# VatsalSy/gerris-fft-particles

Hardware: AMD Instinct MI355X
Metric: Mcell-steps/s (projection+advection), 3D 256^3 uniform (higher is better)
Workload: dtype f64; 1 GPU; 3-D periodic Taylor-Green, 256^3 per GPU, default projection/advection parameters (SURVEY 8d config C); relax_mode=exact, parallelism=1 box, rccl_world_size=0

## Files before the change

gerris-fft-particles_amd/csrc/gfship_internal.hpp:

```cpp
#pragma once

#include <hip/hip_runtime.h>
#include <cstdio>
#include <cstdarg>
#include <cstring>
#include <vector>
#include <deque>
#include <string>
#include <type_traits>
#include "gfship.h"
#include "switches.hpp"
#include "cell_update.hpp"

namespace gfship {

struct Layout {
  int n = 0;
  int px = 0;
  int xo = 1;
  int rows = 0;
  int dim = 3;
  long sy = 0;
  long sz = 0;
  size_t total = 0;
// ... 195 lines not shown
			const RelaxOp * op = nullptr);
int launch_relax_mpi_first (gfship_domain * dom, unsigned dimension, int level, double omega,
			    double * u, const double * rhs, const double * dia, const RelaxOp * op,
			    int (* after_shell) (void *), void * ctx);
void mpi_order_free (gfship_domain * dom);
int launch_relax_loop_small (gfship_domain * dom, unsigned dimension, int level, double omega,
			     Field * dp, Field * ubc, const double * rhs, const double * dia,
			     unsigned nrelax, bool * done, const RelaxOp * op = nullptr);
int coarse_cycle_top (gfship_domain * dom, int minlevel);
int lattice_cycle_top (gfship_domain * dom, int minlevel, Field * dia);
int lattice_check_error (gfship_domain * dom);
int launch_lattice_cycle (gfship_domain * dom, unsigned dimension, double omega, int lmin, int ltop,
			  const unsigned * nrelax, Field * dp, Field * ubc, Field * res);
int launch_coarse_cycle (gfship_domain * dom, unsigned dimension, double omega, int lmin, int ltop,
			 const unsigned * nrelax, Field * dp, Field * ubc, Field * res, Field * dia);
int launch_relax_redblack (gfship_domain * dom, unsigned dimension, int level, double omega,
			   double * u, const double * rhs, const double * dia);
int launch_residual (gfship_domain * dom, int level, const double * u, const double * rhs,
		     const double * dia, double * res);
int launch_residual_weighted (gfship_domain * dom, int level, const double * u, const double * rhs,
			      const double * dia, double * res);
int launch_poisson_weights (gfship_domain * dom, double * const alpha[3]);
int launch_diffusion_weights (gfship_domain * dom, double * const D[3], double cdt);
int alloc_weights (gfship_domain * dom);
RelaxOp weighted_op (gfship_domain * dom, int level);
int launch_restrict (gfship_domain * dom, unsigned dimension, int level_coarse, double * v_coarse,
		     const double * v_fine);
int launch_prolongate (gfship_domain * dom, int level_coarse, const double * v_coarse,
		       double * v_fine);
int launch_correct (gfship_domain * dom, int level, double * u, const double * dp);
int launch_fill (gfship_domain * dom, int level, double * a, double value);
int launch_residual_norm (gfship_domain * dom, int level, const double * u, const double * rhs,
			  const double * dia, double * res, double scale, double weight,
			  double * out , bool dia_zero = false);
int launch_norm_async (gfship_domain * dom, int level, const double * a, double scale, double weight);
int launch_norm (gfship_domain * dom, int level, const double * a, double scale, double weight,
		 double out[5] );

int launch_face_interp_un (gfship_domain * dom, double * const u[3], double * const un[3]);
int launch_divergence (gfship_domain * dom, double * const un[3], double * div, double dt);
int launch_correct_un (gfship_domain * dom, const double * p, double * const un[3], double dt);
int launch_centered_gradient (gfship_domain * dom, const double * p, double * const g[3]);
int launch_correct_centered (gfship_domain * dom, double * const u[3], double * const g[3], double dt);
int launch_correct_centered_coarse (gfship_domain * dom, double * const u[3], double * const g[3],
				    double dt, double * const uc[3]);
int launch_coarse_init_from (gfship_domain * dom, Field * const * v, int nf, int top);
int launch_coarse_init_levels (gfship_domain * dom, Field * const * v, int nf, int top, int bottom);
int launch_advected_face_values (gfship_domain * dom, const double * v, double * const u[3],
				 double * const un[3], double dt, int use_centered, int gradient,
				 double * const fv[6], int cmask, double visc = 0., double gsrc = 0.,
				 const double * msrc = nullptr );
int launch_variable_mac_source (gfship_domain * dom, const double * v, double * const D[3],
				const double * alpha, double * out);
int launch_mac_source_fields (gfship_domain * dom, int c, const double * F, bool add_out, double * out);
int launch_centered_source_fields (gfship_domain * dom, double * v, const double * F, double gsrc, double dt);
int launch_face_bc (gfship_domain * dom, Field * v, double * const fv[6], int cmask);
int launch_predict_un (gfship_domain * dom, int cc, const double * uc, double * const fv[6],
		       double * unc);
int launch_flux_update (gfship_domain * dom, bool velocity, double * v, double * const un[3],
			double * const fv[6], const double * gm, const double * gc, double dt,
			double gsrc = 0.);
int launch_cfl (gfship_domain * dom, double * const u[3], double * const un[3],
		const double visc[3], double * cfl2,
		double * const msrc[3] = nullptr );
int launch_coarse_init (gfship_domain * dom, Field * const * v, int nf);
int launch_velocity_divergence (gfship_domain * dom, double * const u[3], double * out);
bool godunov_fused_supported (const gfship_domain * dom);
bool godunov_fused_mpi_supported (const gfship_domain * dom);
// ... 63 lines not shown
```

gerris-fft-particles_amd/csrc/poisson.hip:

```cpp
#include "gfship_internal.hpp"
#include <cmath>
#include <cfloat>
#include <cstdlib>

using namespace gfship;

#define GFSHIP_CHECK_DIMENSION(dom, d) \
  GFSHIP_CHECK ((d) == (unsigned) (dom)->dim, GFSHIP_EUNSUPPORTED, \
		"dimension %u on a %d-D domain: only the dimension of the domain is implemented", (d), (dom)->dim)

namespace gfship {

static bool weighted_pipelinable (gfship_domain * dom, unsigned dimension, int level)
{
  return dom->relax_mode == GFSHIP_RELAX_EXACT && dimension == 3 && dom->dim == 3 &&
    skew_supported (dom, level) && !dom->force_hyperplane;
}

static bool weighted_pipelined (gfship_domain * dom, unsigned dimension, int level)
{
  return dom->sw.weighted_pipelined && weighted_pipelinable (dom, dimension, level);
}

static int relax_level (gfship_domain * dom, unsigned dimension, int level, double omega,
// ... 84 lines not shown
    if (done)
      return GFSHIP_OK;
  }
  auto sweep = [&] () -> int {
    if (dom->relax_mode == GFSHIP_RELAX_EXACT && dom->has_external) {
      bool done = false;
      int rr = launch_relax_loop_small (dom, dimension, level, omega, dp, u, rhs->lev[level],
					dia->lev[level], 1, &done);
      if (rr || done) return rr;
    }
    return relax_level (dom, dimension, level, omega, dp, rhs, dia);
  };
  if ((r = launch_bc (dom, u, dp, level, 1))) return r;
  for (unsigned n = 0; n < nrelax - 1; n++) {
    if ((r = sweep ())) return r;
    if ((r = launch_bc (dom, u, dp, level, 1))) return r;
  }
  return sweep ();
}

static int norm_residual_finish (gfship_domain * dom, double dt, double s[5], gfship_norm * out);

static int norm_residual (gfship_domain * dom, double dt, Field * res, gfship_norm * out)
{
  const Layout & L = dom->lay[dom->depth];
  double size = 1./L.n;
  double s[5];
  int r = launch_norm (dom, dom->depth, res->lev[dom->depth], 1.*size*size, 1., s);
  if (r) return r;
  return norm_residual_finish (dom, dt, s, out);
}

static int residual_and_norm (gfship_domain * dom, double dt, Field * U, Field * R, Field * D,
			      Field * S, gfship_norm * out)
{
  const int L = dom->depth;
  S->zero[L] = false;
  if (dom->weighted) {
    int rr = launch_residual_weighted (dom, L, U->lev[L], R->lev[L], D->lev[L], S->lev[L]);
    if (rr) return rr;
    return norm_residual (dom, dt, S, out);
  }
  const double size = 1./dom->lay[L].n;
  double s[5];
  int r = launch_residual_norm (dom, L, U->lev[L], R->lev[L], D->lev[L], S->lev[L], 1.*size*size, 1., s,
				D->zero[L]);
  if (r) return r;
  return norm_residual_finish (dom, dt, s, out);
}

static int norm_residual_finish (gfship_domain * dom, double dt, double s[5], gfship_norm * out)
{
  const Layout & L = dom->lay[dom->depth];
  int r;
  double w = (double) ncells (L);
  if (dom->has_external) {
    double sums[5] = { s[0], s[1], s[2], w, s[4] }, mx[1] = { s[3] };
    if ((r = call_reduce_norm (dom, sums, 5, mx))) return r;
    s[0] = sums[0]; s[1] = sums[1]; s[2] = sums[2]; w = sums[3]; s[3] = mx[0]; s[4] = sums[4];
  }
  gfship_norm n;
  n.bias = s[0]; n.first = s[1]; n.second = s[2]; n.infty = s[3]; n.w = w;
  if (n.w > 0.) {
    n.bias /= n.w;
    n.first /= n.w;
    n.second = sqrt (n.second/n.w);
  }
  else
    n.infty = 0.;
  dt *= dt;
  n.bias = s[4]*dt;
  n.first *= dt;
  n.second *= dt;
  n.infty *= dt;
  *out = n;
  return GFSHIP_OK;
}

}
// ... 100 lines not shown
{
  Field * V = get_field (dom, v);
  if (!V || !out) return GFSHIP_EINVAL;
  const Layout & L = dom->lay[dom->depth];
  double size = 1./L.n;
  double vol = dom->dim == 3 ? size*size*size : size*size;
  double s[5];
  int r = launch_norm (dom, dom->depth, V->lev[dom->depth], 1., vol, s);
  if (r) return r;
  gfship_norm n;
  double wv = vol*(double) ncells (L);
  if (dom->has_external) {
    double sums[4] = { s[0], s[1], s[2], wv }, mx[1] = { s[3] };
    if ((r = call_reduce_norm (dom, sums, 4, mx))) return r;
    s[0] = sums[0]; s[1] = sums[1]; s[2] = sums[2]; wv = sums[3]; s[3] = mx[0];
  }
  n.bias = s[0]; n.first = s[1]; n.second = s[2]; n.infty = s[3];
  n.w = wv;
  if (n.w > 0.) {
    n.bias /= n.w;
    n.first /= n.w;
    n.second = sqrt (n.second/n.w);
  }
  else
    n.infty = 0.;
  *out = n;
  return GFSHIP_OK;
}

}

static int poisson_cycle (gfship_domain * dom, gfship_multilevel_params * p,
			  gfship_field u, gfship_field rhs, gfship_field dia, gfship_field res,
			  double dt, gfship_norm * norm)
{
  GFSHIP_CHECK (dom && p, GFSHIP_EINVAL, "null argument");
  GFSHIP_CHECK (p->dimension == 2 || p->dimension == 3, GFSHIP_EINVAL, "dimension must be 2 or 3");
  GFSHIP_CHECK_DIMENSION (dom, p->dimension);
  GFSHIP_CHECK (p->nrelax > 0 && p->erelax > 0, GFSHIP_EINVAL, "nrelax and erelax must be non zero");
  GFSHIP_CHECK (dom->unit_weights, GFSHIP_EINVAL, "call gfship_poisson_coefficients first");
  if (dom->dp_cache < 0)
    dom->dp_cache = gfship_field_alloc (dom, -1);
  gfship_field dpf = dom->dp_cache;
  if (dpf < 0) return dpf;
  Field * U = get_field (dom, u), * R = get_field (dom, rhs), * D = get_field (dom, dia),
    * S = get_field (dom, res), * DP = get_field (dom, dpf);
  int r = GFSHIP_OK;
  bool corrected = false;
  if (!U || !R || !D || !S) return GFSHIP_EINVAL;
  const int L = dom->depth;
  unsigned minlevel = p->minlevel;
  if (minlevel > (unsigned) L) minlevel = L;
  p->depth = L;

#define TRY(x) do { if ((r = (x)) != GFSHIP_OK) goto done; } while (0)
  for (int l = 0; l <= L; l++)
    S->zero[l] = U->zero[l] = false;
  {
    unsigned nrl[GFSHIP_MAXLEVEL + 1];
    {
      unsigned nr = p->nrelax;
      for (int l = L; l >= 0; l--) {
	nrl[l] = nr;
	if (l > (int) minlevel) nr *= p->erelax;
      }
    }
    for (int l = 0; l <= L; l++)
// ... 15 lines not shown
    unsigned first = minlevel;
    if (ltop >= 0) {
      TRY (launch_lattice_cycle (dom, p->dimension, p->omega, (int) minlevel, ltop, nrl, DP, U, S));
      first = ltop + 1;
    }
    else if (ctop >= 0) {
      TRY (launch_coarse_cycle (dom, p->dimension, p->omega, (int) minlevel, ctop, nrl, DP, U, S, D));
      first = ctop + 1;
    }
    else {
      TRY (launch_fill (dom, minlevel, DP->lev[minlevel], 0.));
      TRY (relax_loop (dom, DP, U, p->dimension, minlevel, p->omega, S, D, nrl[minlevel]));
      first = minlevel + 1;
      dom->kc[GFSHIP_KC_COARSE_END_BY_LEVEL]++;
    }
    for (unsigned l = first; l <= p->depth; l++) {
      const bool fp = prolongation_fused (dom, p->dimension, (int) l, nrl[l]) ||
	line_prolongation_fused (dom, p->dimension, (int) l, nrl[l]);
      if (fp) dom->kc[GFSHIP_KC_PROLONGATION_FUSED]++;
      else if (prolongation_fusable (dom, p->dimension, (int) l, nrl[l]) ||
	       line_prolongation_fusable (dom, p->dimension, (int) l, nrl[l]))
	dom->kc[GFSHIP_KC_PROLONGATION_DECLINED]++;
      if (!fp)
	TRY (launch_prolongate (dom, l - 1, DP->lev[l - 1], DP->lev[l]));
      TRY (relax_loop (dom, DP, U, p->dimension, l, p->omega, S, D, nrl[l],
		       (int) l == L ? U->lev[L] : nullptr, &corrected, fp ? DP->lev[l - 1] : nullptr));
    }
  }
  if (!corrected)
    TRY (launch_correct (dom, L, U->lev[L], DP->lev[L]));
  if (!(corrected && all_sides_periodic (dom)))
    TRY (launch_bc (dom, U, U, L, 0));
  if (norm)
    TRY (residual_and_norm (dom, dt, U, R, D, S, norm));
  else if (dom->weighted)
    TRY (launch_residual_weighted (dom, L, U->lev[L], R->lev[L], D->lev[L], S->lev[L]));
  else
    TRY (launch_residual (dom, L, U->lev[L], R->lev[L], D->lev[L], S->lev[L]));
#undef TRY
 done:
  for (int l = 0; l <= L; l++)
    dom->skew[l].rs_ready = false;
  return r;
}

extern "C" {

int gfship_poisson_cycle (gfship_domain * dom, gfship_multilevel_params * p,
			  gfship_field u, gfship_field rhs, gfship_field dia, gfship_field res)
{
  GFSHIP_CHECK (dom != nullptr, GFSHIP_EINVAL, "null domain");
  int r = before_write (dom);
  if (r) return r;
  return poisson_cycle (dom, p, u, rhs, dia, res, 1., nullptr);
}

int gfship_poisson_solve (gfship_domain * dom, gfship_multilevel_params * par,
			  gfship_field lhs, gfship_field rhs, gfship_field res,
			  gfship_field dia, double dt)
{
  GFSHIP_CHECK (dom && par, GFSHIP_EINVAL, "null argument");
  Field * U = get_field (dom, lhs), * R = get_field (dom, rhs), * D = get_field (dom, dia),
    * S = get_field (dom, res);
  if (!U || !R || !D || !S) return GFSHIP_EINVAL;
  GFSHIP_CHECK (par->dimension == 2 || par->dimension == 3, GFSHIP_EINVAL, "dimension must be 2 or 3");
  GFSHIP_CHECK_DIMENSION (dom, par->dimension);
  GFSHIP_CHECK (dom->unit_weights, GFSHIP_EINVAL, "call gfship_poisson_coefficients first");
  { int r = before_write (dom); if (r) return r; }
  int r;
  const int L = dom->depth;
  if ((r = coarse_flush (dom, U, L, true))) return r;
  unsigned minlevel = par->minlevel;
  par->depth = L;
  par->niter = 0;

  bool deferred = par->nitermin >= 1 && par->nitermax >= 1;
  if (deferred) {
    const Layout & Ly = dom->lay[L];
    double size = 1./Ly.n;
    S->zero[L] = false;
    if (dom->weighted) {
      if ((r = launch_residual_weighted (dom, L, U->lev[L], R->lev[L], D->lev[L], S->lev[L]))) return r;
      if ((r = launch_norm_async (dom, L, S->lev[L], 1.*size*size, 1.))) return r;
    }
    else if ((r = launch_residual_norm (dom, L, U->lev[L], R->lev[L], D->lev[L], S->lev[L], 1.*size*size,
					1., nullptr, D->zero[L])))
      return r;
  }
  else {
    if ((r = residual_and_norm (dom, dt, U, R, D, S, &par->residual))) return r;
    par->residual_before = par->residual;
  }

  double res_max_before = par->residual.infty;

  while (par->niter < par->nitermin ||
	 (par->residual.infty > par->tolerance && par->niter < par->nitermax)) {
    if ((r = poisson_cycle (dom, par, lhs, rhs, dia, res, dt, &par->residual))) {
      if (deferred) {
	deferred = false;
	double s0[5];
	if (hipStreamSynchronize (dom->stream) == hipSuccess) {
	  memcpy (s0, dom->h_pinned + 8, sizeof (s0));
	  if (norm_residual_finish (dom, dt, s0, &par->residual_before) == GFSHIP_OK)
	    par->residual = par->residual_before;
	}
	else
	  memset (&par->residual_before, 0, sizeof (par->residual_before)),
	    memset (&par->residual, 0, sizeof (par->residual));
      }
      break;
    }
    if (deferred) {
      deferred = false;
      double s0[5];
      memcpy (s0, dom->h_pinned + 8, sizeof (s0));
      if ((r = norm_residual_finish (dom, dt, s0, &par->residual_before))) break;
      res_max_before = par->residual_before.infty;
    }
    if (par->residual.infty == res_max_before)
      break;
    if (par->residual.infty > res_max_before/1.1 && par->minlevel < par->depth)
      par->minlevel++;
    res_max_before = par->residual.infty;
    par->niter++;
  }

  par->minlevel = minlevel;
  if (r == GFSHIP_OK)
    r = skew_check_error (dom);
  if (r == GFSHIP_OK)
    r = lattice_check_error (dom);
  return r;
}

int gfship_time_relax (gfship_domain * dom, unsigned d, int level, gfship_field u,
		       gfship_field rhs, gfship_field dia, int reps, double * ms_per_sweep)
{
  Field * U = get_field (dom, u), * R = get_field (dom, rhs), * D = get_field (dom, dia);
  if (!U || !R || !D || !ms_per_sweep || reps <= 0) return GFSHIP_EINVAL;
  GFSHIP_CHECK (level >= 0 && level <= dom->depth, GFSHIP_EINVAL, "level %d out of range", level);
  int r;
  if (dom->relax_mode == GFSHIP_RELAX_EXACT && d == 3 && skew_supported (dom, level) &&
      !dom->force_hyperplane) {
    U->zero[level] = false;
    r = skew_time_sweeps (dom, level, U, R->lev[level], D->lev[level], D->zero[level], reps,
			  ms_per_sweep);
    if (r == GFSHIP_OK && dom->sw.skew_stats)
      skew_dump_stats (dom, level);
    return r;
  }
  if ((r = relax_level (dom, d, level, 1., U, R, D))) return r;
  GFSHIP_HIP (hipEventRecord (dom->ev0, dom->stream));
  for (int q = 0; q < reps; q++)
    if ((r = relax_level (dom, d, level, 1., U, R, D))) return r;
  GFSHIP_HIP (hipEventRecord (dom->ev1, dom->stream));
  GFSHIP_HIP (hipEventSynchronize (dom->ev1));
  float ms = 0.f;
  GFSHIP_HIP (hipEventElapsedTime (&ms, dom->ev0, dom->ev1));
  *ms_per_sweep = (double) ms/reps;
  if (dom->sw.skew_stats)
    skew_dump_stats (dom, level);
  return GFSHIP_OK;
}

int gfship_time_relax_loop (gfship_domain * dom, int level, gfship_field u, gfship_field rhs,
			    gfship_field dia, unsigned nrelax, int reps, double * ms_per_loop,
			    int * fused)
// ... 25 lines not shown
```

gerris-fft-particles_amd/csrc/poisson_kernels.hip:

```cpp
#include "gfship_internal.hpp"
#include "cell_loop.hpp"
#include "relax_skew.hpp"
#include <algorithm>
#include <cstdlib>

namespace gfship {

template <int DIM, int OP>
__device__ __forceinline__ double relax_value (const double * __restrict__ u, long c, long sy, long sz,
					       double rhs, double dia, unsigned dimension,
					       double omega, double w, double h2, const W6 * wf = nullptr)
{
  return cell_update<DIM, OP> (kind_weights<OP> (w, ArrayW { wf, c }), ArrayU { u, c, sy, sz }, rhs, dia, u + c,
			       dimension, omega, h2);
}

__device__ __forceinline__ double relax_value_six (const double * __restrict__ u, long c, long sy, long sz,
						    double rhs)
{
  return cell_update_six (ArrayU { u, c, sy, sz }, rhs);
}

template <int DIM, int OP>
__global__ void __launch_bounds__(256)
// ... 273 lines not shown
  const Layout & L = dom->lay[level];
  BcDesc bc;
  for (int d = 0; d < 6; d++) {
    bc.side[d] = dom->side[d];
    bc.type[d] = ubc->bc[d];
    bc.val[d] = nullptr;
  }
  bc.component = ubc->component;
  bc.homogeneous = 1;
  int nface = dom->dim == 3 ? L.n*L.n : L.n;
  int block = nface <= 64 ? 64 : nface <= 256 ? 256 : 1024;
  with_kind ([&] (auto K, auto D3) {
    hipLaunchKernelGGL ((relax_loop_lds_kernel<decltype (D3)::value ? 3 : 2, decltype (K)::value>), dim3 (1),
			dim3 (block), bytes, dom->stream, L, bc, dimension, omega, w, h2, nrelax, dp->lev[level],
			rhs, dia, op_weights (op));
  }, kind, dom->dim == 3);
  GFSHIP_HIP (hipGetLastError ());
  *done = true;
  return GFSHIP_OK;
}

struct CoarseCycleArgs {
  Layout lay[GFSHIP_MAXLEVEL + 1];
  int lmin, ltop;
  unsigned nrelax[GFSHIP_MAXLEVEL + 1];
  double * dp[GFSHIP_MAXLEVEL + 1];
  double * res[GFSHIP_MAXLEVEL + 2];
  const double * dia[GFSHIP_MAXLEVEL + 1];
  BcDesc bc;
  unsigned dimension;
  double omega;
};

template <int DIM>
__global__ void __launch_bounds__(1024)
coarse_cycle_kernel (CoarseCycleArgs A)
{
  extern __shared__ double lds[];
  const int tid = threadIdx.x, nt = blockDim.x;
#ifdef GFSHIP_LAB_CLOCK
  unsigned long long stamp[40]; int nstamp = 0;
#define LAB_STAMP() do { if (nstamp < 40) stamp[nstamp++] = wall_clock64 (); } while (0)
#else
#define LAB_STAMP() do { } while (0)
#endif
  LAB_STAMP ();
  auto lds_off = [&] (int l, int which) -> unsigned {
    unsigned o = 0;
    for (int q = A.lmin; q < l; q++) {
      unsigned r = A.lay[q].n + 2;
      o += 2*(DIM == 3 ? r*r*r : r*r);
    }
    if (which) {
      unsigned r = A.lay[l].n + 2;
      o += DIM == 3 ? r*r*r : r*r;
    }
    return o;
  };
  {
    const unsigned o = lds_off (A.ltop + 1, 0);
    for (size_t q = tid; q < o; q += nt)
      lds[q] = 0.;
  }
  __syncthreads ();
  LAB_STAMP ();
  for (int l = A.ltop; l >= A.lmin; l--) {
    const Layout & Lc = A.lay[l], & Lf = A.lay[l + 1];
    const int n = Lc.n, r = n + 2, rf = 2*n + 2;
    const int ncell = DIM == 3 ? n*n*n : n*n;
    const bool top = l == A.ltop;
    const double * gf = A.res[l + 1];
    const double * sf = lds + (top ? 0 : lds_off (l + 1, 1));
    double * sc = lds + lds_off (l, 1);
    for (int q = tid; q < ncell; q += nt) {
      int i = q % n + 1, j = (q / n) % n + 1, k = DIM == 3 ? q / (n*n) + 1 : 0;
      double val = 0.;
#pragma unroll
      for (int id = 0; id < (1 << DIM); id++) {
	int ci = 2*i - 1 + (id & 1);
	int cj = 2*j - 1 + ((id & 2) ? 0 : 1);
	int ck = DIM == 3 ? 2*k - 1 + ((id & 4) ? 0 : 1) : 0;
	if (top)
	  val += gf[Lf.idx (ci, cj, ck)];
	else
	  val += sf[ci + rf*(cj + (DIM == 3 ? rf*ck : 0))];
      }
      double v = A.dimension == 2 ? val : val/2.;
      sc[i + r*(j + (DIM == 3 ? r*k : 0))] = v;
      A.res[l][Lc.idx (i, j, k)] = v;
    }
    __syncthreads ();
    LAB_STAMP ();
  }
  for (int l = A.lmin; l <= A.ltop; l++) {
    const Layout & L = A.lay[l];
    const int n = L.n, r = n + 2;
    const long ssy = r, ssz = DIM == 3 ? (long) r*r : 0;
    const int ncell = DIM == 3 ? n*n*n : n*n;
    const int nface = DIM == 3 ? n*n : n;
    double * s = (lds + lds_off (l, 0));
    if (l > A.lmin) {
      const int nc = n/2, rc = nc + 2;
      const long cy = rc, cz = DIM == 3 ? (long) rc*rc : 0;
      const double * vc = (lds + lds_off (l - 1, 0));
      for (int q = tid; q < ncell; q += nt) {
	int i = q % n + 1, j = (q / n) % n + 1, k = DIM == 3 ? q / (n*n) + 1 : 0;
	int pi = (i + 1)/2, pj = (j + 1)/2, pk = DIM == 3 ? (k + 1)/2 : 0;
	long p = pi + cy*pj + cz*pk;
	double pv = vc[p];
	double h[3];
	const long off[3] = { 1, cy, cz };
#pragma unroll
	for (int cc = 0; cc < DIM; cc++) {
	  double g1 = vc[p + off[cc]] - 1.*pv;
	  double g2 = vc[p - off[cc]] - 1.*pv;
	  h[cc] = (g1 - g2)/2.;
	}
	double rel[3] = { ((i & 1) ? -1. : 1.)/4., ((j & 1) ? -1. : 1.)/4., ((k & 1) ? -1. : 1.)/4. };
	double val = pv;
#pragma unroll
	for (int cc = 0; cc < DIM; cc++)
	  val += rel[cc]*h[cc];
	s[i + ssy*j + ssz*k] = val;
      }
      __syncthreads ();
    }
    LAB_STAMP ();
    const double * rhs = (lds + lds_off (l, 1));
    const double * dia = A.dia[l];
    const int S = (int) A.nrelax[l];
    if (S > 0) {
      for (int q = tid; q < 2*DIM*nface; q += nt) {
	int d = q / nface, f = q % nface;
	int c = d/2;
	int t1 = f % n + 1, t2 = DIM == 3 ? f / n + 1 : 0;
	int ijk[3] = { 0, 0, 0 };
	int ta = c == 0 ? 1 : 0, tb = c == 2 ? 1 : 2;
	ijk[c] = (d & 1) ? 1 : n;
	ijk[ta] = t1;
	if (DIM == 3) ijk[tb] = t2;
	long o = c == 0 ? 1 : c == 1 ? ssy : ssz;
	if (d & 1) o = - o;
	long nb = ijk[0] + ssy*ijk[1] + ssz*ijk[2];
	double v;
	if (A.bc.side[d] == GFSHIP_SIDE_PERIODIC)
	  v = s[nb - (long) (n - 1)*o];
	else
	  v = ghost_value (A.bc.type[d], A.bc.component, c, s[nb], 1, 0., 0.);
	s[nb + o] = v;
      }
      __syncthreads ();
      const int nplanes = DIM == 3 ? 3*n - 2 : 2*n - 1;
      const int nconc = (nplanes + n - 1)/n;
      const int niter = nplanes + (S - 1)*n;
      const bool per0 = A.bc.side[0] == GFSHIP_SIDE_PERIODIC, per1 = A.bc.side[1] == GFSHIP_SIDE_PERIODIC;
      const bool per2 = A.bc.side[2] == GFSHIP_SIDE_PERIODIC, per3 = A.bc.side[3] == GFSHIP_SIDE_PERIODIC;
      const bool per4 = DIM == 3 && A.bc.side[4] == GFSHIP_SIDE_PERIODIC;
      const bool per5 = DIM == 3 && A.bc.side[5] == GFSHIP_SIDE_PERIODIC;
      const int lg = __ffs (n) - 1, lgf = DIM == 3 ? 2*lg : lg;
      auto cell = [&] (int sw, int I, int J, int K) {
	int i = I + 1, j = n - J, k = DIM == 3 ? n - K : 0;
	long c = i + ssy*j + ssz*k;
	double v;
	if (DIM == 3 && !dia && A.dimension == 3)
	  v = relax_value_six (s, c, ssy, ssz, rhs[c]);
	else {
	  double dv = dia ? dia[L.idx (i, j, k)] : 0.;
	  v = relax_value<DIM, 0> (s, c, ssy, ssz, rhs[c], dv, A.dimension, A.omega, 1., 1.);
	}
	s[c] = v;
	if (sw < S - 1) {
	  if (i == n) {
	    long f = 1 + ssy*j + ssz*k;
	    double first = s[f];
	    s[f - 1] = per1 ? v : ghost_value (A.bc.type[1], A.bc.component, 0, first, 1, 0., 0.);
	    s[c + 1] = per0 ? first : ghost_value (A.bc.type[0], A.bc.component, 0, v, 1, 0., 0.);
	  }
	  if (j == 1) {
	    long f = i + ssy*n + ssz*k;
	    double first = s[f];
	    s[f + ssy] = per2 ? v : ghost_value (A.bc.type[2], A.bc.component, 1, first, 1, 0., 0.);
	    s[c - ssy] = per3 ? first : ghost_value (A.bc.type[3], A.bc.component, 1, v, 1, 0., 0.);
	  }
	  if (DIM == 3 && k == 1) {
	    long f = i + ssy*j + ssz*n;
	    double first = s[f];
	    s[f + ssz] = per4 ? v : ghost_value (A.bc.type[4], A.bc.component, 2, first, 1, 0., 0.);
	    s[c - ssz] = per5 ? first : ghost_value (A.bc.type[5], A.bc.component, 2, v, 1, 0., 0.);
	  }
	}
      };
      if (DIM == 3 && !dia && A.dimension == 3 && nconc*nface <= nt) {
	const int g = tid >> lgf, t = tid & (nface - 1);
	const int J = t & (n - 1), K = t >> lg;
	const int j = n - J, k = n - K;
	double * srow = s + (ssy*j + ssz*k);
	const double * rrow = rhs + (ssy*j + ssz*k);
	double * sj = s + (ssy*n + ssz*k), * sk = s + (ssy*j + ssz*n);
	const bool mine = g < nconc, jl = j == 1, kl = k == 1;
	for (int q = 0; q < niter; q++) {
	  const int sw = min (S - 1, q >> lg) - g;
	  const int I = q - (sw << lg) - J - K;
	  if (mine && sw >= 0 && (unsigned) I < (unsigned) n) {
	    const int i = I + 1;
	    double b = 0.;
	    b += 1.*srow[i + 1];
	    b += 1.*srow[i - 1];
	    b += 1.*srow[i + ssy];
	    b += 1.*srow[i - ssy];
	    b += 1.*srow[i + ssz];
	    b += 1.*srow[i - ssz];
	    const double v = divide_by_6 (b - rrow[i]);
	    srow[i] = v;
	    if (sw < S - 1 && (i == n || jl || kl)) {
	      if (i == n) {
		double first = srow[1];
		srow[0] = per1 ? v : ghost_value (A.bc.type[1], A.bc.component, 0, first, 1, 0., 0.);
		srow[n + 1] = per0 ? first : ghost_value (A.bc.type[0], A.bc.component, 0, v, 1, 0., 0.);
	      }
	      if (jl) {
		double first = sj[i];
		sj[i + ssy] = per2 ? v : ghost_value (A.bc.type[2], A.bc.component, 1, first, 1, 0., 0.);
		srow[i - ssy] = per3 ? first : ghost_value (A.bc.type[3], A.bc.component, 1, v, 1, 0., 0.);
	      }
	      if (kl) {
// ... 520 lines not shown
  int i = 2*ih + 1 + ((j + k + colour) & 1);
  if (i > n) return;
  long c = L.idx (i, j, k);
  u[c] = relax_value<DIM, 0> (u, c, L.sy, L.sz, rhs[c], dia[c], dimension, omega, 1., 1.);
}

int launch_relax_redblack (gfship_domain * dom, unsigned dimension, int level, double omega,
			   double * u, const double * rhs, const double * dia)
{
  const Layout & L = dom->lay[level];
  int half = (L.n + 1)/2;
  int block = half >= 128 ? 128 : 64;
  dim3 grid ((half + block - 1)/block, L.n, dom->dim == 3 ? L.n : 1);
  for (int colour = 0; colour < 2; colour++) {
    with_bools ([&] (auto D3) {
      hipLaunchKernelGGL (relax_redblack_kernel<decltype (D3)::value ? 3 : 2>, grid, dim3 (block), 0, dom->stream,
			  L, colour, dimension, omega, u, rhs, dia);
    }, dom->dim == 3);
  }
  GFSHIP_HIP (hipGetLastError ());
  return GFSHIP_OK;
}

template <int DIM>
__global__ void __launch_bounds__(256)
residual_kernel (Layout L, const double * __restrict__ u, const double * __restrict__ rhs,
		 const double * __restrict__ dia, double * __restrict__ res)
{
  CELL_LOOP_PROLOGUE (L);
  const FaceSums s = face_sums<DIM> (UnitW {}, ArrayU { u, c, L.sy, L.sz }, dia[c]);
  res[c] = residual_close (s.a, s.b, rhs[c], u[c]);
}

template <bool NORM>
__global__ void residual_norm2_kernel (Layout L, const double * __restrict__ u, const double * __restrict__ rhs,
				       const double * __restrict__ dia, double * __restrict__ res, double inv,
				       double weight, double * __restrict__ partial);

int launch_residual (gfship_domain * dom, int level, const double * u, const double * rhs,
		     const double * dia, double * res)
{
  const Layout & L = dom->lay[level];
  dim3 grid, block;
  cell_grid (L, &grid, &block);
  const bool pairs = dom->sw.residual_pairs;
  if (dom->dim == 3 && L.n >= 64) dom->kc[pairs ? GFSHIP_KC_RESIDUAL_PAIRS : GFSHIP_KC_RESIDUAL_SCALAR]++;
  if (dom->dim == 3 && L.n >= 64 && pairs) {
    const long nitems = (long) L.n*L.n*(L.n/2);
    long nb = (nitems + 255)/256;
    if (nb > 4096) nb = 4096;
    hipLaunchKernelGGL (residual_norm2_kernel<false>, dim3 ((int) nb), dim3 (256), 0, dom->stream, L, u, rhs,
			dia, res, 1., 1., nullptr);
    GFSHIP_HIP (hipGetLastError ());
    return GFSHIP_OK;
  }
  with_bools ([&] (auto D3) {
    hipLaunchKernelGGL (residual_kernel<decltype (D3)::value ? 3 : 2>, grid, block, 0, dom->stream, L, u, rhs, dia, res);
  }, dom->dim == 3);
  GFSHIP_HIP (hipGetLastError ());
  return GFSHIP_OK;
}

template <int DIM>
__global__ void __launch_bounds__(256)
residual_weighted_kernel (Layout L, const double * __restrict__ u, const double * __restrict__ rhs,
			  const double * __restrict__ dia, double * __restrict__ res, W6 wf)
{
// ... 365 lines not shown
  memcpy (out, dom->h_pinned, 5*sizeof (double));
  return GFSHIP_OK;
}

template <int DIM>
__global__ void __launch_bounds__(256)
residual_norm_kernel (Layout L, const double * __restrict__ u, const double * __restrict__ rhs,
		      const double * __restrict__ dia, double * __restrict__ res, double inv,
		      double weight, double * __restrict__ partial)
{
  const int n = L.n;
  const long nrows = DIM == 3 ? (long) n*n : n;
  double s0 = 0., s1 = 0., s2 = 0., s3 = 0., s4 = 0.;
  for (long r = blockIdx.x; r < nrows; r += gridDim.x) {
    const int j = (int) (r % n) + 1, k = DIM == 3 ? (int) (r / n) + 1 : 0;
    const long row = L.idx (1, j, k);
    for (int i = threadIdx.x; i < n; i += blockDim.x) {
      const long c = row + i;
      const FaceSums f = face_sums<DIM> (UnitW {}, ArrayU { u, c, L.sy, L.sz }, dia ? dia[c] : 0.);
      const double raw = residual_close (f.a, f.b, rhs[c], u[c]);
      res[c] = raw;
      double val = raw*inv;
      s0 += weight*val;
      val = fabs (val);
      s3 = fmax (s3, val);
      s1 += weight*val;
      s2 += weight*val*val;
      s4 += raw;
    }
  }
  block_norm_sums (s0, s1, s2, s3, s4, partial, blockIdx.x);
}

template <bool NORM>
__global__ void __launch_bounds__(256)
residual_norm2_kernel (Layout L, const double * __restrict__ u, const double * __restrict__ rhs,
		       const double * __restrict__ dia, double * __restrict__ res, double inv,
		       double weight, double * __restrict__ partial)
{
  typedef double d2 __attribute__((ext_vector_type(2)));
  const int n = L.n, half = n >> 1;
  const long nitems = (long) n*n*half;
  double s0 = 0., s1 = 0., s2 = 0., s3 = 0., s4 = 0.;
  for (long it = (long) blockIdx.x*blockDim.x + threadIdx.x; it < nitems; it += (long) gridDim.x*blockDim.x) {
    const int pr = (int) (it % half);
    const long r = it / half;
    const int j = (int) (r % n) + 1, k = (int) (r / n) + 1;
    const long c = L.idx (1 + 2*pr, j, k);
    const d2 uc = *(const d2 *) (u + c);
    const double ul = u[c - 1], ur = u[c + 2];
    const d2 ut = *(const d2 *) (u + c + L.sy), ub = *(const d2 *) (u + c - L.sy);
    const d2 uf = *(const d2 *) (u + c + L.sz), uk = *(const d2 *) (u + c - L.sz);
    const d2 rh = *(const d2 *) (rhs + c);
    d2 di = { 0., 0. };
    if (dia) di = *(const d2 *) (dia + c);
    d2 out;
    {
      double a = di.x, b = 0.;
      a += 1.; b += 1.*uc.y;
      a += 1.; b += 1.*ul;
      a += 1.; b += 1.*ut.x;
      a += 1.; b += 1.*ub.x;
      a += 1.; b += 1.*uf.x;
      a += 1.; b += 1.*uk.x;
      out.x = rh.x - (b - uc.x*a);
    }
    {
      double a = di.y, b = 0.;
      a += 1.; b += 1.*ur;
      a += 1.; b += 1.*uc.x;
      a += 1.; b += 1.*ut.y;
      a += 1.; b += 1.*ub.y;
      a += 1.; b += 1.*uf.y;
      a += 1.; b += 1.*uk.y;
      out.y = rh.y - (b - uc.y*a);
    }
    *(d2 *) (res + c) = out;
    if (NORM)
#pragma unroll
    for (int e = 0; e < 2; e++) {
      const double raw = e ? out.y : out.x;
      double val = raw*inv;
      s0 += weight*val;
      val = fabs (val);
      s3 = fmax (s3, val);
      s1 += weight*val;
      s2 += weight*val*val;
      s4 += raw;
    }
  }
  if (!NORM) return;
  __shared__ double sh[5][4];
  s0 = wave_sum (s0); s1 = wave_sum (s1); s2 = wave_sum (s2); s3 = wave_max (s3); s4 = wave_sum (s4);
  int w = threadIdx.x >> 6, lane = threadIdx.x & 63;
  if (lane == 0) { sh[0][w] = s0; sh[1][w] = s1; sh[2][w] = s2; sh[3][w] = s3; sh[4][w] = s4; }
  __syncthreads ();
  if (threadIdx.x == 0) {
    int nw = blockDim.x >> 6;
    double r0 = 0., r1 = 0., r2 = 0., r3 = 0., r4 = 0.;
    for (int q = 0; q < nw; q++) {
      r0 += sh[0][q]; r1 += sh[1][q]; r2 += sh[2][q]; r3 = fmax (r3, sh[3][q]); r4 += sh[4][q];
    }
    double * p = partial + 5*(size_t) blockIdx.x;
    p[0] = r0; p[1] = r1; p[2] = r2; p[3] = r3; p[4] = r4;
  }
}

int launch_residual_norm (gfship_domain * dom, int level, const double * u, const double * rhs,
			  const double * dia, double * res, double scale, double weight,
			  double * out, bool dia_zero)
{
  const Layout & L = dom->lay[level];
  if (!power_of_two (scale)) {
    int r = launch_residual (dom, level, u, rhs, dia, res);
    if (r) return r;
    return out ? launch_norm (dom, level, res, scale, weight, out) :
      launch_norm_async (dom, level, res, scale, weight);
  }
  long nrows = L.dim == 3 ? (long) L.n*L.n : L.n;
  int block = L.n >= 256 ? 256 : L.n >= 128 ? 128 : 64;
  int rn_blocks = dom->sw.rn_blocks;
  if (rn_blocks < 64 || rn_blocks > 8192) rn_blocks = 4096;
  int nblocks = (int) (nrows > rn_blocks ? rn_blocks : nrows);
  double * partial = dom->d_scratch;
  double * result = out ? dom->h_pinned : dom->h_pinned + 8;
  const bool rn_pairs = dom->sw.residual_pairs;
  if (dom->dim == 3 && L.n >= 64) dom->kc[rn_pairs ? GFSHIP_KC_RESIDUAL_PAIRS : GFSHIP_KC_RESIDUAL_SCALAR]++;
  if (dom->dim == 3 && L.n >= 64 && rn_pairs) {
    const long nitems = (long) L.n*L.n*(L.n/2);
    long nb = (nitems + 255)/256;
    nblocks = (int) (nb > rn_blocks ? rn_blocks : nb);
    hipLaunchKernelGGL (residual_norm2_kernel<true>, dim3 (nblocks), dim3 (256), 0, dom->stream, L, u,
			rhs, dia_zero ? nullptr : dia, res, 1./scale, weight, partial);
  }
  else
    with_bools ([&] (auto D3) {
      hipLaunchKernelGGL (residual_norm_kernel<decltype (D3)::value ? 3 : 2>, dim3 (nblocks), dim3 (block), 0,
			  dom->stream, L, u, rhs, dia_zero ? nullptr : dia, res, 1./scale, weight, partial);
    }, dom->dim == 3);
  hipLaunchKernelGGL (norm_final_kernel, dim3 (1), dim3 (256), 0, dom->stream,
		      partial, nblocks, result);
  GFSHIP_HIP (hipGetLastError ());
  dom->kc[GFSHIP_KC_RN_BLOCKS_LIMIT] = rn_blocks;
  if ((unsigned long long) nblocks > dom->kc[GFSHIP_KC_RN_BLOCKS_MAX])
    dom->kc[GFSHIP_KC_RN_BLOCKS_MAX] = nblocks;
  if (out) {
    GFSHIP_HIP (stream_wait_spin (dom->stream));
    memcpy (out, dom->h_pinned, 5*sizeof (double));
  }
  return GFSHIP_OK;
}

struct MpiOrderPlan {
  int * cells = nullptr;
  std::vector<int> first;
  int shell_steps = 0;
};

template <int DIM, int OP>
__global__ void __launch_bounds__(256)
relax_listed_kernel (const int * __restrict__ cells, int count, long sy, long sz,
		     unsigned dimension, double omega, double w, double h2,
		     double * __restrict__ u, const double * __restrict__ rhs,
		     const double * __restrict__ dia)
{
  const int q = blockIdx.x*blockDim.x + threadIdx.x;
// ... 141 lines not shown
```

gerris-fft-particles_amd/csrc/simulation.hip:

```cpp
#include "gfship_internal.hpp"
#include <cmath>
#include <cfloat>
#include <cstdlib>

using namespace gfship;

#define G_MAXINT 2147483647

struct gfship_sim {
  gfship_domain * dom = nullptr;
  gfship_field p = -1, pmac = -1, u[3] = {-1, -1, -1}, g[3] = {-1, -1, -1}, gmac[3] = {-1, -1, -1};
  std::vector<gfship_field> tracers;
  std::vector<int> tracer_gradient;
  std::vector<int> tracer_scheme;
  std::vector<double> tracer_D;
  std::deque<gfship_multilevel_params> tracer_diffusion_params;
  bool tracer_diffusion_fused = true;
  unsigned long long tracer_diffusion_counts[2] = { 0, 0 };
  gfship_field un[3] = {-1, -1, -1};
  gfship_field fv[6] = {-1, -1, -1, -1, -1, -1};
  gfship_field dia = -1, div = -1, res = -1, tmp = -1;
  gfship_multilevel_params projection_params, approx_projection_params;
  gfship_advection_params advection_params;
  double t = 0., end = DBL_MAX, dtmax = DBL_MAX, tnext = 0.;
// ... 140 lines not shown
		    const gfship_field g[3], bool approximate = false, bool lazy = false)
{
  gfship_domain * dom = s->dom;
  double * un[3], * gp[3], * u[3];
  ptrs3 (s, s->un, un);
  ptrs3 (s, g, gp);
  ptrs3 (s, s->u, u);
  if (s->has_alpha) {
    TRY (gfship_poisson_coefficients_alpha (dom, s->alpha));
    lazy = false;
  }
  else
    TRY (gfship_poisson_coefficients (dom));
  for (int l = 0; l <= dom->depth; l++)
    if (!dom->fields[s->dia].zero[l])
      TRY (gfship_field_fill (dom, s->dia, l, 0.));
  for (int c = 0; c < dom->dim; c++)
    if (has_viscosity (s, c) || dom->src[c] != 0. || s->has_srcf) lazy = false;
  if (!approximate || !s->tracers.empty () || s->un_handle_given || p != s->p || !dom->sw.lazy_un)
    lazy = false;
  if (!approximate)
    TRY (materialize_un (s));
  else
    s->un_lazy = false;
  if (approximate)
    TRY (launch_face_interp_div (dom, u, lazy ? nullptr : un, leaf (s, s->div), dt));
  else if (!(s->div_ready && s->div_dt == dt)) {
    TRY (launch_divergence (dom, un, leaf (s, s->div), dt));
    dom->kc[GFSHIP_KC_DIVERGENCE_SEPARATE]++;
  }
  else
    dom->kc[GFSHIP_KC_DIVERGENCE_FUSED]++;
  s->div_ready = false;
  TRY (gfship_poisson_solve (dom, par, p, s->div, s->res, s->dia, dt));
  s->cfl_ready = false;
  bool want_max = approximate, ghosts_done = false;
  for (int c = 0; c < dom->dim; c++)
    if (has_viscosity (s, c) || dom->src[c] != 0. || s->has_srcf) want_max = false;
  if (s->has_alpha) {
    want_max = false;
    TRY (launch_project_correct_weighted (dom, leaf (s, p), un, gp, approximate ? u : nullptr, dt));
  }
  else if (lazy) {
    const int L = dom->depth;
    double * uo[3];
    for (int c = 0; c < dom->dim; c++) {
      if (s->adv_tmp3[c] < 0)
	s->adv_tmp3[c] = gfship_field_alloc (dom, -1);
      if (s->adv_tmp3[c] < 0) return s->adv_tmp3[c];
    }
    ptrs3 (s, s->adv_tmp3, uo);
    TRY (launch_project_correct_lazy (dom, leaf (s, p), u, gp, uo, dt, &ghosts_done));
    for (int c = 0; c < dom->dim; c++) {
      std::swap (dom->fields[s->u[c]].lev[L], dom->fields[s->adv_tmp3[c]].lev[L]);
      dom->fields[s->u[c]].zero[L] = false;
    }
    s->un_lazy = true;
    s->un_lazy_dt = dt;
  }
  else
    TRY (launch_project_correct (dom, leaf (s, p), un, gp, approximate ? u : nullptr, dt, want_max, &ghosts_done));
  s->cfl_ready = want_max;
  if (!ghosts_done)
    TRY (bc_leaf_vector (s, g));
  if (approximate && !(ghosts_done && lazy))
    TRY (bc_leaf_vector (s, s->u));
  return GFSHIP_OK;
// ... 888 lines not shown
```

Before: 2892 Mcell-steps/s.

## Skip residual store on predicted final cycle and specialize coarse plane sweep

The projection solve now predicts its final V-cycle from the previous iteration count and, on that cycle, launches a residual-norm kernel variant that skips writing the fine residual field, since the simulation never reads it afterwards. If the prediction is wrong and another cycle runs, the residual is recomputed explicitly first. The change also adds a templated coarse plane-wavefront relaxation loop for small power-of-two coarse grids, and a vectorised top-level restriction in the coarse cycle kernel. Together these remove one full-grid store of the residual per solve and cut index arithmetic in the coarse solver. In exchange the code is more complex and pays an extra residual launch whenever the iteration count changes.

```diff
diff --git a/gerris-fft-particles_amd/csrc/gfship_internal.hpp b/gerris-fft-particles_amd/csrc/gfship_internal.hpp
--- a/gerris-fft-particles_amd/csrc/gfship_internal.hpp
+++ b/gerris-fft-particles_amd/csrc/gfship_internal.hpp
@@ -251,8 +251,12 @@
 int launch_fill (gfship_domain * dom, int level, double * a, double value);
 int launch_residual_norm (gfship_domain * dom, int level, const double * u, const double * rhs,
 			  const double * dia, double * res, double scale, double weight,
-			  double * out , bool dia_zero = false);
+			  double * out , bool dia_zero = false,
+			  bool * store = nullptr );
 int launch_norm_async (gfship_domain * dom, int level, const double * a, double scale, double weight);
+
+int poisson_solve (gfship_domain * dom, gfship_multilevel_params * par, gfship_field lhs, gfship_field rhs,
+		   gfship_field res, gfship_field dia, double dt, bool res_unread);
 int launch_norm (gfship_domain * dom, int level, const double * a, double scale, double weight,
 		 double out[5] );
 
diff --git a/gerris-fft-particles_amd/csrc/poisson.hip b/gerris-fft-particles_amd/csrc/poisson.hip
--- a/gerris-fft-particles_amd/csrc/poisson.hip
+++ b/gerris-fft-particles_amd/csrc/poisson.hip
@@ -140,8 +140,9 @@
 }
 
 static int residual_and_norm (gfship_domain * dom, double dt, Field * U, Field * R, Field * D,
-			      Field * S, gfship_norm * out)
-{
+			      Field * S, gfship_norm * out, bool * store = nullptr)
+{
+  if (store && dom->weighted) *store = true;
   const int L = dom->depth;
   S->zero[L] = false;
   if (dom->weighted) {
@@ -152,7 +153,7 @@
   const double size = 1./dom->lay[L].n;
   double s[5];
   int r = launch_residual_norm (dom, L, U->lev[L], R->lev[L], D->lev[L], S->lev[L], 1.*size*size, 1., s,
-				D->zero[L]);
+				D->zero[L], store);
   if (r) return r;
   return norm_residual_finish (dom, dt, s, out);
 }
@@ -319,7 +320,7 @@
 
 static int poisson_cycle (gfship_domain * dom, gfship_multilevel_params * p,
 			  gfship_field u, gfship_field rhs, gfship_field dia, gfship_field res,
-			  double dt, gfship_norm * norm)
+			  double dt, gfship_norm * norm, bool * store_res = nullptr)
 {
   GFSHIP_CHECK (dom && p, GFSHIP_EINVAL, "null argument");
   GFSHIP_CHECK (p->dimension == 2 || p->dimension == 3, GFSHIP_EINVAL, "dimension must be 2 or 3");
@@ -401,7 +402,7 @@
   if (!(corrected && all_sides_periodic (dom)))
     TRY (launch_bc (dom, U, U, L, 0));
   if (norm)
-    TRY (residual_and_norm (dom, dt, U, R, D, S, norm));
+    TRY (residual_and_norm (dom, dt, U, R, D, S, norm, store_res));
   else if (dom->weighted)
     TRY (launch_residual_weighted (dom, L, U->lev[L], R->lev[L], D->lev[L], S->lev[L]));
   else
@@ -427,6 +428,17 @@
 int gfship_poisson_solve (gfship_domain * dom, gfship_multilevel_params * par,
 			  gfship_field lhs, gfship_field rhs, gfship_field res,
 			  gfship_field dia, double dt)
+{
+  return poisson_solve (dom, par, lhs, rhs, res, dia, dt, false);
+}
+
+}
+
+namespace gfship {
+
+int poisson_solve (gfship_domain * dom, gfship_multilevel_params * par,
+		   gfship_field lhs, gfship_field rhs, gfship_field res,
+		   gfship_field dia, double dt, bool res_unread)
 {
   GFSHIP_CHECK (dom && par, GFSHIP_EINVAL, "null argument");
   Field * U = get_field (dom, lhs), * R = get_field (dom, rhs), * D = get_field (dom, dia),
@@ -441,6 +453,8 @@
   if ((r = coarse_flush (dom, U, L, true))) return r;
   unsigned minlevel = par->minlevel;
   par->depth = L;
+  const unsigned predicted = res_unread ? par->niter : 0;
+  bool res_stored = true;
   par->niter = 0;
 
   bool deferred = par->nitermin >= 1 && par->nitermax >= 1;
@@ -465,7 +479,14 @@
 
   while (par->niter < par->nitermin ||
 	 (par->residual.infty > par->tolerance && par->niter < par->nitermax)) {
-    if ((r = poisson_cycle (dom, par, lhs, rhs, dia, res, dt, &par->residual))) {
+    if (!res_stored) {
+      if ((r = launch_residual (dom, L, U->lev[L], R->lev[L], D->lev[L], S->lev[L]))) break;
+      res_stored = true;
+    }
+    bool store = !(predicted > 0 && par->niter + 1 == predicted);
+    r = poisson_cycle (dom, par, lhs, rhs, dia, res, dt, &par->residual, &store);
+    res_stored = store;
+    if (r) {
       if (deferred) {
 	deferred = false;
 	double s0[5];
@@ -503,6 +524,10 @@
   return r;
 }
 
+}
+
+extern "C" {
+
 int gfship_time_relax (gfship_domain * dom, unsigned d, int level, gfship_field u,
 		       gfship_field rhs, gfship_field dia, int reps, double * ms_per_sweep)
 {
diff --git a/gerris-fft-particles_amd/csrc/poisson_kernels.hip b/gerris-fft-particles_amd/csrc/poisson_kernels.hip
--- a/gerris-fft-particles_amd/csrc/poisson_kernels.hip
+++ b/gerris-fft-particles_amd/csrc/poisson_kernels.hip
@@ -329,6 +329,65 @@
   double omega;
 };
 
+template <int LG, bool PER>
+__device__ __forceinline__ void coarse_plane_loop (double * s, const BcDesc & bc, const int S, const int tid)
+{
+  constexpr int n = 1 << LG, r = n + 2, ssy = r, ssz = r*r, nface = n*n;
+  constexpr int nplanes = 3*n - 2, nconc = (nplanes + n - 1)/n;
+  const int niter = nplanes + (S - 1)*n;
+  const bool per0 = PER || bc.side[0] == GFSHIP_SIDE_PERIODIC, per1 = PER || bc.side[1] == GFSHIP_SIDE_PERIODIC;
+  const bool per2 = PER || bc.side[2] == GFSHIP_SIDE_PERIODIC, per3 = PER || bc.side[3] == GFSHIP_SIDE_PERIODIC;
+  const bool per4 = PER || bc.side[4] == GFSHIP_SIDE_PERIODIC, per5 = PER || bc.side[5] == GFSHIP_SIDE_PERIODIC;
+  const int g = tid >> (2*LG), t = tid & (nface - 1);
+  const int J = t & (n - 1), K = t >> LG;
+  const int j = n - J, k = n - K;
+  double * srow = s + (ssy*j + ssz*k);
+  const double * rrow = srow + r*r*r;
+  const bool jl = j == 1, kl = k == 1;
+  const double * fyrow = srow + (jl ? (n - 1)*ssy : 0), * fzrow = srow + (kl ? (n - 1)*ssz : 0);
+  const int none = 1 << 30;
+  int q0 = g < nconc && g < S ? g*n + J + K : none;
+  const int qlim = S*n + J + K;
+  const int rlim = (S - 1)*n + J + K;
+  for (int q = 0; q < niter; q++) {
+    const int I = q - q0;
+    if ((unsigned) I < (unsigned) n) {
+      const int i = I + 1;
+      const double right = srow[i + 1], left = srow[i - 1], up = srow[i + ssy], down = srow[i - ssy];
+      const double front = srow[i + ssz], back = srow[i - ssz], rh = rrow[i];
+      const double fx = srow[1], fy = fyrow[i], fz = fzrow[i];
+      double b = 0.;
+      b += 1.*right;
+      b += 1.*left;
+      b += 1.*up;
+      b += 1.*down;
+      b += 1.*front;
+      b += 1.*back;
+      const double v = divide_by_6 (b - rh);
+      srow[i] = v;
+      if (q0 < rlim) {
+	if (i == n) {
+	  srow[0] = per1 ? v : ghost_value (bc.type[1], bc.component, 0, fx, 1, 0., 0.);
+	  srow[n + 1] = per0 ? fx : ghost_value (bc.type[0], bc.component, 0, v, 1, 0., 0.);
+	}
+	if (jl) {
+	  srow[i + n*ssy] = per2 ? v : ghost_value (bc.type[2], bc.component, 1, fy, 1, 0., 0.);
+	  srow[i - ssy] = per3 ? fy : ghost_value (bc.type[3], bc.component, 1, v, 1, 0., 0.);
+	}
+	if (kl) {
+	  srow[i + n*ssz] = per4 ? v : ghost_value (bc.type[4], bc.component, 2, fz, 1, 0., 0.);
+	  srow[i - ssz] = per5 ? fz : ghost_value (bc.type[5], bc.component, 2, v, 1, 0., 0.);
+	}
+      }
+      if (i == n) {
+	q0 += nconc*n;
+	if (q0 >= qlim) q0 = none;
+      }
+    }
+    __syncthreads ();
+  }
+}
+
 template <int DIM>
 __global__ void __launch_bounds__(1024)
 coarse_cycle_kernel (CoarseCycleArgs A)
@@ -369,6 +428,42 @@
     const double * gf = A.res[l + 1];
     const double * sf = lds + (top ? 0 : lds_off (l + 1, 1));
     double * sc = lds + lds_off (l, 1);
+    if (DIM == 3 && top) {
+      typedef double d2 __attribute__((ext_vector_type(2)));
+      const int lgc = __ffs (n) - 1;
+      for (int q0 = tid; q0 < ncell; q0 += 4*nt) {
+	d2 ch[4][4];
+#pragma unroll
+	for (int e = 0; e < 4; e++) {
+	  const int q = q0 + e*nt;
+	  if (q < ncell) {
+	    const int i = (q & (n - 1)) + 1, j = ((q >> lgc) & (n - 1)) + 1, k = (q >> 2*lgc) + 1;
+	    const double * p = gf + Lf.idx (2*i - 1, 2*j, 2*k);
+	    ch[e][0] = *(const d2 *) p;
+	    ch[e][1] = *(const d2 *) (p - Lf.sy);
+	    ch[e][2] = *(const d2 *) (p - Lf.sz);
+	    ch[e][3] = *(const d2 *) (p - Lf.sy - Lf.sz);
+	  }
+	}
+#pragma unroll
+	for (int e = 0; e < 4; e++) {
+	  const int q = q0 + e*nt;
+	  if (q < ncell) {
+	    const int i = (q & (n - 1)) + 1, j = ((q >> lgc) & (n - 1)) + 1, k = (q >> 2*lgc) + 1;
+	    double val = 0.;
+#pragma unroll
+	    for (int m = 0; m < 4; m++) {
+	      val += ch[e][m].x;
+	      val += ch[e][m].y;
+	    }
+	    double v = A.dimension == 2 ? val : val/2.;
+	    sc[i + r*(j + r*k)] = v;
+	    A.res[l][Lc.idx (i, j, k)] = v;
+	  }
+	}
+      }
+    }
+    else
     for (int q = tid; q < ncell; q += nt) {
       int i = q % n + 1, j = (q / n) % n + 1, k = DIM == 3 ? q / (n*n) + 1 : 0;
       double val = 0.;
@@ -431,14 +526,13 @@
 	int d = q / nface, f = q % nface;
 	int c = d/2;
 	int t1 = f % n + 1, t2 = DIM == 3 ? f / n + 1 : 0;
-	int ijk[3] = { 0, 0, 0 };
-	int ta = c == 0 ? 1 : 0, tb = c == 2 ? 1 : 2;
-	ijk[c] = (d & 1) ? 1 : n;
-	ijk[ta] = t1;
-	if (DIM == 3) ijk[tb] = t2;
+	const int fixed = (d & 1) ? 1 : n;
+	const int ci = c == 0 ? fixed : t1;
+	const int cj = c == 1 ? fixed : c == 0 ? t1 : t2;
+	const int ck = DIM == 3 ? (c == 2 ? fixed : t2) : 0;
 	long o = c == 0 ? 1 : c == 1 ? ssy : ssz;
 	if (d & 1) o = - o;
-	long nb = ijk[0] + ssy*ijk[1] + ssz*ijk[2];
+	long nb = ci + ssy*cj + ssz*ck;
 	double v;
 	if (A.bc.side[d] == GFSHIP_SIDE_PERIODIC)
 	  v = s[nb - (long) (n - 1)*o];
@@ -447,6 +541,7 @@
 	s[nb + o] = v;
       }
       __syncthreads ();
+      LAB_STAMP ();
       const int nplanes = DIM == 3 ? 3*n - 2 : 2*n - 1;
       const int nconc = (nplanes + n - 1)/n;
       const int niter = nplanes + (S - 1)*n;
@@ -487,7 +582,27 @@
 	  }
 	}
       };
-      if (DIM == 3 && !dia && A.dimension == 3 && nconc*nface <= nt) {
+      bool looped = false;
+      if constexpr (DIM == 3)
+	if (!dia && A.dimension == 3 && nconc*nface <= nt && lg >= 2 && lg <= 4) {
+	  const bool per = per0 && per1 && per2 && per3 && per4 && per5;
+	  if (per)
+	    switch (lg) {
+	    case 2: coarse_plane_loop<2, true> (s, A.bc, S, tid); break;
+	    case 3: coarse_plane_loop<3, true> (s, A.bc, S, tid); break;
+	    default: coarse_plane_loop<4, true> (s, A.bc, S, tid); break;
+	    }
+	  else
+	    switch (lg) {
+	    case 2: coarse_plane_loop<2, false> (s, A.bc, S, tid); break;
+	    case 3: coarse_plane_loop<3, false> (s, A.bc, S, tid); break;
+	    default: coarse_plane_loop<4, false> (s, A.bc, S, tid); break;
+	    }
+	  looped = true;
+	}
+      if (looped)
+	;
+      else if (DIM == 3 && !dia && A.dimension == 3 && nconc*nface <= nt) {
 	const int g = tid >> lgf, t = tid & (nface - 1);
 	const int J = t & (n - 1), K = t >> lg;
 	const int j = n - J, k = n - K;
@@ -1074,7 +1189,7 @@
   res[c] = residual_close (s.a, s.b, rhs[c], u[c]);
 }
 
-template <bool NORM>
+template <bool NORM, bool STORE = true>
 __global__ void residual_norm2_kernel (Layout L, const double * __restrict__ u, const double * __restrict__ rhs,
 				       const double * __restrict__ dia, double * __restrict__ res, double inv,
 				       double weight, double * __restrict__ partial);
@@ -1506,7 +1621,7 @@
   block_norm_sums (s0, s1, s2, s3, s4, partial, blockIdx.x);
 }
 
-template <bool NORM>
+template <bool NORM, bool STORE>
 __global__ void __launch_bounds__(256)
 residual_norm2_kernel (Layout L, const double * __restrict__ u, const double * __restrict__ rhs,
 		       const double * __restrict__ dia, double * __restrict__ res, double inv,
@@ -1549,7 +1664,8 @@
       a += 1.; b += 1.*uk.y;
       out.y = rh.y - (b - uc.y*a);
     }
-    *(d2 *) (res + c) = out;
+    if (STORE)
+      *(d2 *) (res + c) = out;
     if (NORM)
 #pragma unroll
     for (int e = 0; e < 2; e++) {
@@ -1582,9 +1698,12 @@
 
 int launch_residual_norm (gfship_domain * dom, int level, const double * u, const double * rhs,
 			  const double * dia, double * res, double scale, double weight,
-			  double * out, bool dia_zero)
+			  double * out, bool dia_zero, bool * store)
 {
   const Layout & L = dom->lay[level];
+  const bool no_store = store && !*store && power_of_two (scale) && dom->dim == 3 && L.n >= 64 &&
+    dom->sw.residual_pairs;
+  if (store) *store = !no_store;
   if (!power_of_two (scale)) {
     int r = launch_residual (dom, level, u, rhs, dia, res);
     if (r) return r;
@@ -1604,8 +1723,10 @@
     const long nitems = (long) L.n*L.n*(L.n/2);
     long nb = (nitems + 255)/256;
     nblocks = (int) (nb > rn_blocks ? rn_blocks : nb);
-    hipLaunchKernelGGL (residual_norm2_kernel<true>, dim3 (nblocks), dim3 (256), 0, dom->stream, L, u,
-			rhs, dia_zero ? nullptr : dia, res, 1./scale, weight, partial);
+    with_bools ([&] (auto ST) {
+      hipLaunchKernelGGL ((residual_norm2_kernel<true, decltype (ST)::value>), dim3 (nblocks), dim3 (256), 0,
+			  dom->stream, L, u, rhs, dia_zero ? nullptr : dia, res, 1./scale, weight, partial);
+    }, !no_store);
   }
   else
     with_bools ([&] (auto D3) {
diff --git a/gerris-fft-particles_amd/csrc/simulation.hip b/gerris-fft-particles_amd/csrc/simulation.hip
--- a/gerris-fft-particles_amd/csrc/simulation.hip
+++ b/gerris-fft-particles_amd/csrc/simulation.hip
@@ -196,7 +196,7 @@
   else
     dom->kc[GFSHIP_KC_DIVERGENCE_FUSED]++;
   s->div_ready = false;
-  TRY (gfship_poisson_solve (dom, par, p, s->div, s->res, s->dia, dt));
+  TRY (poisson_solve (dom, par, p, s->div, s->res, s->dia, dt, true));
   s->cfl_ready = false;
   bool want_max = approximate, ghosts_done = false;
   for (int c = 0; c < dom->dim; c++)
```

New measurement: 2932 Mcell-steps/s, median of 6. 1.4% higher.
